# h3poteto/aws-global-accelerator-controller

Hardware: NVIDIA H100
Metric: objects reconciled/sec at 10^6 Service+Ingress; change-set bit-exact vs Go ref (higher is better)
Workload: dtype u8/u32 (bytes and indices)

## Files before the change

aws-global-accelerator-controller_b200/csrc/gar_common.h:

```cpp
#pragma once

#include <stdint.h>
#include <stddef.h>

#include "../../include/garecon.h"

#if defined(__CUDACC__)
#define GAR_HD __host__ __device__ __forceinline__
#define GAR_D __device__ __forceinline__
#else
#define GAR_HD inline
#define GAR_D inline
#endif

#if defined(__CUDA_ARCH__)
#define GAR_ANY(p) __any_sync(0xffffffffu, (p))
#else
bool gar_host_vote(bool p);
#define GAR_ANY(p) gar_host_vote((p))
#endif

typedef uint8_t u8;
typedef uint16_t u16;
typedef uint32_t u32;
// ... 102 lines not shown
#define XXP2 0xC2B2AE3D27D4EB4Full
#define XXP3 0x165667B19E3779F9ull
#define XXP4 0x85EBCA77C2B2AE63ull
#define XXP5 0x27D4EB2F165667C5ull

GAR_HD u64 rotl64(u64 x, int r) { return (x << r) | (x >> (64 - r)); }
GAR_HD u64 xx_round(u64 acc, u64 in) { return rotl64(acc + in * XXP2, 31) * XXP1; }
GAR_HD u64 xx_merge(u64 acc, u64 v) { return (acc ^ xx_round(0, v)) * XXP1 + XXP4; }
GAR_HD u64 xx_avalanche(u64 h) {
  h ^= h >> 33;
  h *= XXP2;
  h ^= h >> 29;
  h *= XXP3;
  h ^= h >> 32;
  return h;
}

GAR_HD u64 hash_init(u32 n) { return XXP5 ^ ((u64)n * XXP3); }
GAR_HD u64 hash_word(u64 h, u64 w) { return rotl64(h ^ (w * XXP2), 31) * XXP1 + XXP4; }
GAR_HD u64 load_word(Str s, u32 i) {
  u64 w = ld64u(s.p + i);
  if (s.n - i < 8) w &= lowmask(s.n - i);
  return w;
}
GAR_HD u64 gar_hash(Str s) {
  u64 h = hash_init(s.n);
  for (u32 i = 0; i < s.n; i += 8) h = hash_word(h, load_word(s, i));
  return xx_avalanche(h);
}

GAR_HD u64 u_hash(bool act, Str s) {
  u64 h = hash_init(s.n);
  const u32 n = act ? s.n : 0;
  for (u32 i = 0;; i += 8) {
    bool step = i < n;
    if (!GAR_ANY(step)) break;
    if (step) h = hash_word(h, load_word(s, i));
  }
  return xx_avalanche(h);
}
GAR_HD bool u_streq(bool act, Str a, Str b) {
  bool eq = act && a.n == b.n;
  const u32 n = eq ? a.n : 0;
  for (u32 i = 0;; i += 8) {
    bool step = eq && i < n;
    if (!GAR_ANY(step)) break;
    if (step) {
      u64 x = ld64u(a.p + i) ^ ld64u(b.p + i);
      if (n - i < 8) x &= lowmask(n - i);
      if (x) eq = false;
    }
  }
  return eq;
}
GAR_HD u32 u_find_byte(bool act, Str s, u32 from, u8 c) {
  u32 found = s.n;
  bool done = !act;
  for (u32 i = from;; i += 8) {
    bool step = !done && i < s.n;
    if (!GAR_ANY(step)) break;
    if (!step) continue;
    u64 m = swar_eq_mask(ld64u(s.p + i), c);
    if (s.n - i < 8) m &= lowmask(s.n - i);
    if (m) {
      found = i + (ctz64(m) >> 3);
      done = true;
    }
  }
  return found;
}

GAR_HD u64 hmix(u64 a, u64 b) { return xx_avalanche(a * XXP1 + rotl64(b, 29) * XXP2 + XXP5); }


struct alignas(32) IdxEntry {
  u32 tag, row, a0, a1;
  u64 s0, s1;
};

struct HashIdx {
  const u32 *begin;
  const IdxEntry *ent;
  u32 mask;
};

struct Cursor {
  u32 pos, end, tag;
};

GAR_HD u32 hash_bucket(u64 h, u32 mask) { return (u32)h & mask; }
GAR_HD u32 hash_tag(u64 h) { return (u32)(h >> 32); }

GAR_HD IdxEntry load_entry(const IdxEntry *p) {
#if defined(__CUDA_ARCH__)
  const uint4 *q = reinterpret_cast<const uint4 *>(p);
  uint4 lo = __ldg(q), hi = __ldg(q + 1);
  IdxEntry e;
  e.tag = lo.x;
  e.row = lo.y;
  e.a0 = lo.z;
  e.a1 = lo.w;
  e.s0 = (u64)hi.x | ((u64)hi.y << 32);
  e.s1 = (u64)hi.z | ((u64)hi.w << 32);
  return e;
#else
  return *p;
#endif
}

GAR_HD Cursor idx_open(const HashIdx &ix, u64 h) {
  u32 b = hash_bucket(h, ix.mask);
  Cursor c;
  c.pos = ix.begin[b];
  c.end = ix.begin[b + 1];
  c.tag = hash_tag(h);
  return c;
}
GAR_HD bool idx_next(const HashIdx &ix, Cursor &c, IdxEntry *out) {
  while (c.pos < c.end) {
    IdxEntry e = load_entry(ix.ent + c.pos++);
    if (e.tag == c.tag) {
      *out = e;
      return true;
    }
  }
  return false;
}
```

aws-global-accelerator-controller_b200/csrc/gar_pipeline.h:

```cpp
#pragma once

#include <stdio.h>
#include <stdlib.h>

#include <initializer_list>

#include "gar_rows.h"

#if defined(__CUDA_ARCH__)
#define GAR_ATOMIC_ADD(p, v) atomicAdd((p), (v))
#else
#define GAR_ATOMIC_ADD(p, v) (*(p) += (v))
#endif


enum Slot {
  S_DERIVED, S_OFLAGS, S_OKEY_HASH, S_STAGE_GA, S_STAGE_R53, S_ANN_R53, S_ANN_NAME, S_ANN_TAGS, S_ANN_LISTEN, S_DPORT_BEGIN, S_DPORTS,
  S_TOK_CODE, S_TOK_NAME, S_TOK_REGION,
  S_ACC_FLAGS, S_ACC_OWNER_KEY, S_ACC_OWNER, S_ACC_THOST, S_ACC_MANAGED, S_ACC_OWNER_HASH, S_ACC_THOST_HASH, S_REC_NAME_HASH, S_VAL_KEY_HASH,
  S_REC_ZONE, S_VAL_REC, S_VAL_CLS, S_VAL_KEY, S_VAL_ORPHAN, S_VAL_LINK, S_ACC_DIGEST,
  S_R53_MODE, S_R53_ACC, S_R53_ACC_DNS, S_PAIR_BEGIN, S_PAIR_OBJ, S_PAIR_HN, S_PAIR_CODE, S_PAIR_ZONE, S_PAIR_REC,
  S_IX_LB, S_IX_OWNER = S_IX_LB + 3, S_IX_THOST = S_IX_OWNER + 3, S_IX_ZONE = S_IX_THOST + 3, S_IX_VAL = S_IX_ZONE + 3,
  S_IX_ALIAS = S_IX_VAL + 3, S_IX_OBJ = S_IX_ALIAS + 3, S_IX_OVN = S_IX_OBJ + 3,
  S_SORT_KEYS = S_IX_OVN + 3, S_SORT_VALS, S_SORT_KEYS_ALT, S_SORT_VALS_ALT, S_SORT_TAGS,
// ... 283 lines not shown
    e->a1 = W.rec_zone[rec];
    e->s0 = T.a.rec_name[rec];
    e->s1 = T.a.val_value[v];
    return W.val_orphan[v] != 0;
  }
};

constexpr u32 IDX_SMALL_BUCKET = 48;
template <class RowF>
struct FIdxRows {
  RowF rowf;
  u32 *keys, *vals;
  IdxEntry *tmp;
  u32 *counts;
  u32 mask, nb;
  GAR_HD void operator()(u32 i) const {
    u64 h = 0;
    IdxEntry e;
    bool valid = rowf.make(i, &h, &e);
    u32 k = valid ? hash_bucket(h, mask) : nb;
    keys[i] = k;
    if (vals) vals[i] = i;
    if (valid) {
      e.tag = hash_tag(h);
      e.row = i;
      tmp[i] = e;
      GAR_ATOMIC_ADD(&counts[k], 1u);
    }
  }
};
struct FIdxPlace {
  const u32 *keys;
  u32 *cursor;
  const IdxEntry *tmp;
  IdxEntry *ent;
  u32 nb;
  GAR_HD void operator()(u32 i) const {
    u32 k = keys[i];
    if (k == nb) return;
#if defined(__CUDA_ARCH__)
    u32 pos = atomicAdd(&cursor[k], 1u);
#else
    u32 pos = cursor[k]++;
#endif
    ent[pos] = tmp[i];
  }
};
struct FIdxOrder {
  const u32 *begin;
  IdxEntry *ent;
  u32 *overflow;
  GAR_HD void operator()(u32 b) const {
    u32 lo = begin[b], m = begin[b + 1] - lo;
    if (m < 2) return;
    if (m > IDX_SMALL_BUCKET) {
      GAR_ATOMIC_ADD(overflow, 1u);
      return;
    }
    for (u32 k = 1; k < m; k++) {
      IdxEntry x = ent[lo + k];
      u32 j = k;
      while (j > 0 && ent[lo + j - 1].row > x.row) {
        ent[lo + j] = ent[lo + j - 1];
        j--;
      }
      if (j != k) ent[lo + j] = x;
    }
  }
};
struct FIdxGather {
  const u32 *vals;
  const u32 *nvalid;
  const IdxEntry *tmp;
  IdxEntry *ent;
  GAR_HD void operator()(u32 p) const {
    if (p < *nvalid) ent[p] = tmp[vals[p]];
  }
};
template <class RowF>
struct FIdxPlaceDirect {
  RowF rowf;
  u32 *cursor;
  IdxEntry *ent;
  u32 mask;
  GAR_HD void operator()(u32 i) const {
    u64 h = 0;
    IdxEntry e;
    if (!rowf.make(i, &h, &e)) return;
    const u32 k = hash_bucket(h, mask);
#if defined(__CUDA_ARCH__)
    const u32 pos = atomicAdd(&cursor[k], 1u);
#else
    const u32 pos = cursor[k]++;
#endif
    e.tag = hash_tag(h);
    e.row = i;
    ent[pos] = e;
  }
};
struct FIdxMultiList {
  const u32 *begin;
  u32 *multi;
  GAR_HD void operator()(u32 b) const {
    const bool m = begin[b + 1] - begin[b] >= 2;
#if defined(__CUDA_ARCH__)
    const unsigned active = __activemask();
    const unsigned votes = __ballot_sync(active, m);
    if (!m) return;
    const unsigned lane = threadIdx.x & 31u;
    const int leader = __ffs(votes) - 1;
    u32 base = 0;
    if ((int)lane == leader) base = atomicAdd(multi, (u32)__popc(votes));
    base = __shfl_sync(votes, base, leader);
    multi[1 + base + __popc(votes & ((1u << lane) - 1u))] = b;
#else
    if (m) multi[1 + multi[0]++] = b;
#endif
  }
};
struct FIdxOrderMulti {
  const u32 *begin;
  IdxEntry *ent;
  const u32 *multi;
  u32 *overflow;
  GAR_HD void operator()(u32 t) const {
    const u32 b = multi[1 + t];
    const u32 lo = begin[b], m = begin[b + 1] - lo;
    if (m > IDX_SMALL_BUCKET) {
      GAR_ATOMIC_ADD(overflow, 1u);
      return;
    }
    for (u32 k = 1; k < m; k++) {
      IdxEntry x = ent[lo + k];
      u32 j = k;
      while (j > 0 && ent[lo + j - 1].row > x.row) {
        ent[lo + j] = ent[lo + j - 1];
        j--;
      }
      if (j != k) ent[lo + j] = x;
    }
  }
};
enum FlagWord { FW_BAD_KEYS = 0, FW_IDX_OVERFLOW = 1, FW_NDPORTS = 2, FW_NPAIRS = 3, FW_SEC0 = 4 , FW_WORDS = 16 };
struct FGatherFinal {
  const u32 *src;
  u32 idx[5];
  const u32 *npairs;
  u32 *flags;
  GAR_HD void operator()(u32 k) const {
    if (k < 5) flags[FW_SEC0 + k] = src[idx[k]];
    else if (npairs) flags[FW_NPAIRS] = *npairs;
  }
};
struct FGather5 {
  const u32 *src;
  u32 idx[5];
  const u32 *extra;
  u32 *dst;
  GAR_HD void operator()(u32 k) const { dst[k] = k < 5 ? src[idx[k]] : *extra; }
};
#define GAR_RETRY_WITH_RADIX 1000
#define GAR_REFUSE_EMPTY_CACHE 1001
struct FGatherHeader {
  const u32 *ndports;
  u32 *flags;
  GAR_HD void operator()(u32) const { flags[FW_NDPORTS] = *ndports; }
};
struct FValueJoins {
  DevTables T;
  Work W;
  GAR_HD void operator()(u32 v) const {
    link_value_alias(T, W, v);
    mark_orphan_value(T, W, v);
  }
};
struct FMarkOrphanValue {
  DevTables T;
  Work W;
  GAR_HD void operator()(u32 v) const { mark_orphan_value(T, W, v); }
};

struct CountLayout {
  u32 n, nacc, nrec, nval;
  GAR_HD u32 ga_obj(u32 i) const { return i; }
  GAR_HD u32 ga_orph(u32 a) const { return n + a; }
  GAR_HD u32 r53_obj(u32 i) const { return n + nacc + i; }
  GAR_HD u32 base0() const { return 2 * n + nacc; }
  GAR_HD u32 base1() const { return 2 * n + nacc + nrec; }
  GAR_HD u32 total() const { return 2 * n + nacc + nrec + nval; }
};
constexpr u32 OPS_STAGE_CAP = 4;
struct FGaObj {
  DevTables T;
  Work W;
  u32 *counts;
  gar_op *stage;
  u32 *status;
  const u32 *rows;
  GAR_HD void operator()(u32 t, bool valid) const {
    u32 i = (rows && valid) ? rows[t] : t;
    OpSink s{stage + (size_t)t * OPS_STAGE_CAP, 0, OPS_STAGE_CAP};
    u32 st = ga_reconcile(T, W, i, valid, s);
    if (valid) {
      status[t] = st;
      counts[t] = s.n;
    }
  }
};
struct FR53Obj {
  DevTables T;
  Work W;
  u32 *counts;
  gar_op *stage;
  u32 *status;
  const u32 *rows;
  GAR_HD void operator()(u32 t, bool valid) const {
    u32 i = (rows && valid) ? rows[t] : t;
    OpSink s{stage + (size_t)t * OPS_STAGE_CAP, 0, OPS_STAGE_CAP};
    u32 prev = (valid && W.r53_mode[i] == R53_MODE_DONE) ? status[t] : 0;
    u32 st = r53_combine(T, W, i, t, valid, prev, s);
    if (valid) {
      status[t] = st;
      counts[t] = s.n;
// ... 151 lines not shown
    u32 zv = T.a.rec_val_begin[T.a.zone_rec_begin[z]];
    u32 off = counts[L.base0()] + (counts[L.base1() + zv] - counts[L.base1()]) + (counts[L.base0() + r] - counts[L.base0()]);
    OpSink s{ops + off, 0, 0xFFFFFFFFu};
    r53_orphan_alias(T, W, r, s);
  }
};
struct FR53OrphanValue {
  DevTables T;
  Work W;
  CountLayout L;
  u32 *counts;
  gar_op *ops;
  u32 cap;
  GAR_HD void operator()(u32 v) const {
    if (!ops) {
      counts[L.base1() + v] = W.val_orphan[v];
      return;
    }
    if (!W.val_orphan[v] || counts[L.total()] > cap) return;
    u32 r = W.val_rec[v];
    u32 z = W.rec_zone[r];
    u32 rend = T.a.zone_rec_begin[z + 1];
    u32 off = counts[L.base0()] + (counts[L.base0() + rend] - counts[L.base0()]) + (counts[L.base1() + v] - counts[L.base1()]);
    gar_op o;
    o.head = GAR_OP_HEAD(GAR_OP_R53_DELETE_RECORD, GAR_CTRL_R53, 0);
    o.obj = GAR_NONE;
    o.sub = 1;
    o.a0 = z;
    o.a1 = r;
    o.a2 = v;
    ops[off] = o;
  }
};


struct DiffCounts {
  u64 n_ops;
  u64 section_begin[GAR_N_SECTIONS + 1];
  u64 n_dports;
  u32 bad_keys;
};

GAR_HD u32 next_pow2(u32 x) {
  u32 p = 1;
  while (p < x) p <<= 1;
  return p;
}
inline int ilog2(u32 p) {
  int b = 0;
  while ((1u << b) < p) b++;
  return b;
}

template <class B>
struct Pipeline {
  B &be;
  DevTables T;
  Work W{};
  bool force_radix = false;
  explicit Pipeline(B &b, const DevTables &t) : be(b), T(t) {}

  template <class RowF>
  HashIdx build_index(int slot, u32 nrows, u32 load, RowF rowf, u32 *overflow, bool force_radix) {
    u32 nb = next_pow2(nrows / load < 16 ? 16 : nrows / load);
    u32 *keys = (u32 *)be.ensure(S_SORT_KEYS, sizeof(u32) * (size_t)(nrows + 1));
    u32 *vals = (u32 *)be.ensure(S_SORT_VALS, sizeof(u32) * (size_t)(nrows + 1));
    IdxEntry *tmp = (IdxEntry *)be.ensure(S_SORT_TAGS, sizeof(IdxEntry) * (size_t)(nrows + 1));
    u32 *begin = (u32 *)be.ensure(slot + 0, sizeof(u32) * (size_t)(nb + 2));
    IdxEntry *ent = (IdxEntry *)be.ensure(slot + 1, sizeof(IdxEntry) * (size_t)(nrows + 1));
    be.fill32(begin, 0, nb + 2);
    if (nrows) be.for_each("idx_rows", nrows, FIdxRows<RowF>{rowf, keys, force_radix ? vals : nullptr, tmp, begin, nb - 1, nb});
    be.exclusive_scan(begin, nb + 2);
    if (nrows && !force_radix) {
      u32 *cursor = (u32 *)be.ensure(S_SORT_KEYS_ALT, sizeof(u32) * (size_t)(nb + 1));
      be.copy32(cursor, begin, nb);
      be.for_each("idx_place", nrows, FIdxPlace{keys, cursor, tmp, ent, nb});
      be.for_each("idx_order", nb, FIdxOrder{begin, ent, overflow});
    } else if (nrows) {
      u32 *keys2 = (u32 *)be.ensure(S_SORT_KEYS_ALT, sizeof(u32) * (size_t)(nrows + 1));
      u32 *vals2 = (u32 *)be.ensure(S_SORT_VALS_ALT, sizeof(u32) * (size_t)(nrows + 1));
      be.sort_pairs(keys, vals, keys2, vals2, nrows, ilog2(nb) + 1);
      be.for_each("idx_gather", nrows, FIdxGather{vals, begin + nb, tmp, ent});
    }
    return HashIdx{begin, ent, nb - 1};
  }

  bool prepared = false;
  u64 n_dports = 0;
  u32 *errflag = nullptr;

  u32 acc_guest_from = 0xFFFFFFFFu;
  u32 sharded = 0;
  bool orphan_sweep = true;
  bool allow_empty_cache = false;

  void alloc_obj_work() {
    const u32 n = T.o.n_objects, nlbi = T.o.n_lbi;
    W.derived = (u32 *)be.ensure(S_DERIVED, 4 * (size_t)(n + 1));
    W.okey_hash = (u64 *)be.ensure(S_OKEY_HASH, 8 * (size_t)(n + 1));
    W.ann_r53 = (gar_str *)be.ensure(S_ANN_R53, 8 * (size_t)(n + 1));
    W.ann_name = (gar_str *)be.ensure(S_ANN_NAME, 8 * (size_t)(n + 1));
    W.ann_tags = (gar_str *)be.ensure(S_ANN_TAGS, 8 * (size_t)(n + 1));
    W.ann_listen = (gar_str *)be.ensure(S_ANN_LISTEN, 8 * (size_t)(n + 1));
    W.dport_begin = (u32 *)be.out_dport_begin(n);
    W.tok_code = (u8 *)be.out_tok_code(nlbi);
    W.tok_name = (gar_str *)be.out_tok_name(nlbi);
    W.tok_region = (gar_str *)be.out_tok_region(nlbi);
    W.r53_mode = (u8 *)be.ensure(S_R53_MODE, (size_t)n + 1);
    W.r53_acc = (u32 *)be.ensure(S_R53_ACC, 4 * (size_t)(n + 1));
    W.r53_acc_dns = (gar_str *)be.ensure(S_R53_ACC_DNS, 8 * (size_t)(n + 1));
  }
  void alloc_work() {
    const u32 nacc = T.a.n_accels, nrec = T.a.n_records, nval = T.a.n_values;
    alloc_obj_work();
    W.acc_flags = (u32 *)be.ensure(S_ACC_FLAGS, 4 * (size_t)(nacc + 1));
    W.acc_owner_key = (gar_str *)be.ensure(S_ACC_OWNER_KEY, 8 * (size_t)(nacc + 1));
    W.acc_owner = (gar_str *)be.ensure(S_ACC_OWNER, 8 * (size_t)(nacc + 1));
    W.acc_thost = (gar_str *)be.ensure(S_ACC_THOST, 8 * (size_t)(nacc + 1));
    W.acc_managed = (gar_str *)be.ensure(S_ACC_MANAGED, 8 * (size_t)(nacc + 1));
    W.acc_owner_hash = (u64 *)be.ensure(S_ACC_OWNER_HASH, 8 * (size_t)(nacc + 1));
    W.acc_thost_hash = (u64 *)be.ensure(S_ACC_THOST_HASH, 8 * (size_t)(nacc + 1));
    W.rec_name_hash = (u64 *)be.ensure(S_REC_NAME_HASH, 8 * (size_t)(nrec + 1));
    W.val_key_hash = (u64 *)be.ensure(S_VAL_KEY_HASH, 8 * (size_t)(nval + 1));
    W.rec_zone = (u32 *)be.ensure(S_REC_ZONE, 4 * (size_t)(nrec + 1));
    W.val_rec = (u32 *)be.ensure(S_VAL_REC, 4 * (size_t)(nval + 1));
    W.val_cls = (u8 *)be.ensure(S_VAL_CLS, nval + 1);
    W.val_key = (gar_str *)be.ensure(S_VAL_KEY, 8 * (size_t)(nval + 1));
    W.val_orphan = (u8 *)be.ensure(S_VAL_ORPHAN, nval + 1);
    W.val_link = (ValLink *)be.ensure(S_VAL_LINK, sizeof(ValLink) * (size_t)(nval + 1));
    W.acc_digest = (AccDigest *)be.ensure(S_ACC_DIGEST, sizeof(AccDigest) * (size_t)(nacc + 1));
    W.lb_hash = (u64 *)be.ensure(S_LB_HASH, 8 * (size_t)(T.a.n_lbs + 1));
    W.rec_flags = (u8 *)be.ensure(S_REC_FLAGS, (size_t)nrec + 1);
    for (int k = 0; k < IX_N; k++) W.hist[k] = IxHist{nullptr, 0};
    W.pair_cap = 0;
    W.dport_cap = 0;
    errflag = (u32 *)be.ensure(S_ERRFLAG, 256);
    be.fill32(errflag, 0, FW_WORDS);
    W.acc_guest_from = acc_guest_from;
    W.sharded = sharded;
    W.acc_claimed = nullptr;
  }
  void stage1() {
    const u32 n = T.o.n_objects, nlbi = T.o.n_lbi, nacc = T.a.n_accels, nrec = T.a.n_records, nval = T.a.n_values;
    u32 *derived_public = (u32 *)be.out_derived(n);
    if (n) be.for_each("classify_objects", n, FClassify{T, W, derived_public, nullptr, errflag});
    if (nlbi) be.for_each_staged("tokenise_hostnames", nlbi, FTokenise{T, W});
    if (nacc) be.for_each("digest_accelerators", nacc, FDigestAccel{T, W});
    if (T.a.n_lbs) be.for_each("hash_load_balancers", T.a.n_lbs, FLbHash{T, W});
    {
      unsigned long long *zm = (unsigned long long *)(errflag + 16 + 8);
      be.fill32((u32 *)zm, 0, 8);
      if (T.a.n_zones) be.for_each("zone_len_mask", T.a.n_zones, FZoneLenMask{T, W, zm});
      W.zone_len_mask = (const u64 *)zm;
    }
    if (nrec) {
      u32 *big = (u32 *)be.ensure(S_SORT_KEYS, 4 * (size_t)(nval / REC_INLINE_VALUES + 2));
      u32 *huge = (u32 *)be.ensure(S_SORT_VALS, 4 * (size_t)(nval / REC_HUGE_VALUES + 2));
      be.fill32(big, 0, 1);
      be.fill32(huge, 0, 1);
      be.for_each_staged("prepare_records", nrec, FPrepareRecord{T, W, big, huge});
      if (nval > REC_INLINE_VALUES) be.for_each("prepare_records", BIG_BLOCKS * 256, FClassifyBigRecords{T, W, big, huge});
    }
  }
  struct IxPlan {
    u32 off[IX_N] = {}, nb[IX_N] = {}, rows[IX_N] = {};
    bool want[IX_N] = {};
    u32 total_nb = 0;
    u64 total_rows = 0;
  };
  IxPlan planA;
  u32 *ixa_begin = nullptr, *ixa_fill = nullptr, *ixa_multi = nullptr;
  IdxEntry *ixa_ent = nullptr;
  u32 ovn_nb = 0;
  void arm_group_a(u32 want_mask) {
    const u32 rows[IX_N] = {T.a.n_lbs, T.a.n_accels, T.a.n_accels, T.a.n_zones, T.a.n_values, T.a.n_records, T.o.n_objects, 0};
    const u32 load[IX_N] = {1, 1, 1, 1, 1, 2, 1, 8};
    planA = IxPlan{};
    for (int k = 0; k < IX_OVN; k++) {
      planA.want[k] = (want_mask >> k) & 1u;
      if (!planA.want[k]) continue;
      planA.rows[k] = rows[k];
      planA.nb[k] = next_pow2(rows[k] / load[k] < 16 ? 16 : rows[k] / load[k]);
      planA.off[k] = planA.total_nb;
      planA.total_nb += planA.nb[k];
      planA.total_rows += rows[k];
    }
    ixa_begin = (u32 *)be.ensure(S_IXA_BEGIN, 4 * (size_t)(planA.total_nb + 2));
    be.fill32(ixa_begin, 0, (size_t)planA.total_nb + 2);
    for (int k = 0; k < IX_OVN; k++)
      if (planA.want[k]) W.hist[k] = IxHist{ixa_begin + planA.off[k], planA.nb[k] - 1};
  }
  HashIdx group_a_index(int k) const { return HashIdx{ixa_begin + planA.off[k], ixa_ent, planA.nb[k] - 1}; }
  template <class RowF>
  FIdxPlaceDirect<RowF> placer(int k, RowF rowf) const {
    return FIdxPlaceDirect<RowF>{rowf, ixa_fill + planA.off[k], ixa_ent, planA.nb[k] - 1};
  }
  void finish_group_a() {
    u32 *overflow = errflag + FW_IDX_OVERFLOW;
    be.exclusive_scan(ixa_begin, planA.total_nb + 1);
    ixa_fill = (u32 *)be.ensure(S_IXA_FILL, 4 * (size_t)(planA.total_nb + 1));
    ixa_ent = (IdxEntry *)be.ensure(S_IXA_ENT, sizeof(IdxEntry) * (size_t)(planA.total_rows + 1));
    const u32 multi_cap = (u32)(planA.total_rows / 2 + 1);
    ixa_multi = (u32 *)be.ensure(S_IXA_MULTI, 4 * (size_t)(multi_cap + 2));
    be.copy32(ixa_fill, ixa_begin, (size_t)planA.total_nb + 1);
    be.fill32(ixa_multi, 0, 1);
    const IxPlan &P = planA;
    auto n = [&](int k) { return P.want[k] ? P.rows[k] : 0u; };
    be.for_each_multi("idx_place", {n(IX_LB), n(IX_OWNER), n(IX_THOST), n(IX_ZONE), n(IX_VAL), n(IX_ALIAS), n(IX_OBJ), P.total_nb},
                      placer(IX_LB, FRowLb{T, W}), placer(IX_OWNER, FRowOwner{T, W}), placer(IX_THOST, FRowThost{T, W}), placer(IX_ZONE, FRowZone{T}),
                      placer(IX_VAL, FRowVal{T, W}), placer(IX_ALIAS, FRowAlias{T, W}), placer(IX_OBJ, FRowObj{T, W}), FIdxMultiList{ixa_begin, ixa_multi});
    be.for_each_dyn("idx_order", ixa_multi, multi_cap, FIdxOrderMulti{ixa_begin, ixa_ent, ixa_multi, overflow});
    if (P.want[IX_LB]) W.ix_lb = group_a_index(IX_LB);
    if (P.want[IX_OWNER]) W.ix_owner = group_a_index(IX_OWNER);
    if (P.want[IX_THOST]) W.ix_thost = group_a_index(IX_THOST);
    if (P.want[IX_ZONE]) W.ix_zone = group_a_index(IX_ZONE);
    if (P.want[IX_VAL]) W.ix_val = group_a_index(IX_VAL);
    if (P.want[IX_ALIAS]) W.ix_alias = group_a_index(IX_ALIAS);
    if (P.want[IX_OBJ]) W.ix_obj = group_a_index(IX_OBJ);
  }
  void arm_ovn() {
    ovn_nb = next_pow2(T.a.n_values / 8 < 16 ? 16 : T.a.n_values / 8);
    u32 *cnt = (u32 *)be.ensure(S_IX_OVN + 0, 4 * (size_t)(ovn_nb + 2));
    be.fill32(cnt, 0, (size_t)ovn_nb + 2);
    W.hist[IX_OVN] = IxHist{cnt, ovn_nb - 1};
  }
  void finish_ovn() {
    const u32 nval = T.a.n_values;
    u32 *begin = W.hist[IX_OVN].cnt;
    be.exclusive_scan(begin, ovn_nb + 1);
    u32 *cursor = (u32 *)be.ensure(S_OVN_FILL, 4 * (size_t)(ovn_nb + 1));
    IdxEntry *ent = (IdxEntry *)be.ensure(S_IX_OVN + 1, sizeof(IdxEntry) * (size_t)(nval + 1));
    u32 *multi = (u32 *)be.ensure(S_OVN_MULTI, 4 * (size_t)(nval / 2 + 3));
    be.copy32(cursor, begin, (size_t)ovn_nb + 1);
    be.fill32(multi, 0, 1);
    be.for_each_multi("idx_place", {nval, ovn_nb}, FIdxPlaceDirect<FRowOvn>{FRowOvn{T, W}, cursor, ent, ovn_nb - 1}, FIdxMultiList{begin, multi});
    be.for_each_dyn("idx_order", multi, nval / 2 + 1, FIdxOrderMulti{begin, ent, multi, errflag + FW_IDX_OVERFLOW});
    W.ix_ovn = HashIdx{begin, ent, ovn_nb - 1};
  }

  void prepare_route() {
    alloc_work();
    arm_group_a(1u << IX_ALIAS);
    stage1();
    finish_group_a();
  }
  void prepare_directory() {
    alloc_work();
    arm_group_a((1u << IX_LB) | (1u << IX_THOST));
    if (T.o.n_lbi) be.for_each("tokenise_hostnames", T.o.n_lbi, FTokenise{T, W});
    if (T.a.n_accels) be.for_each("digest_accelerators", T.a.n_accels, FDigestAccel{T, W});
    if (T.a.n_lbs) be.for_each("hash_load_balancers", T.a.n_lbs, FLbHash{T, W});
    finish_group_a();
  }

  u32 dport_cap = 0, pair_cap = 0;
  u64 ops_cap = 0;
  bool tiny_caps = false;
  int prepare() {
    const u32 n = T.o.n_objects, nacc = T.a.n_accels, nzone = T.a.n_zones, nrec = T.a.n_records, nval = T.a.n_values;
    alloc_work();
    if (!force_radix) {
      arm_group_a((1u << IX_OVN) - 1);
      arm_ovn();
    }
    stage1();
    listen_ports();

    u32 *overflow = errflag + FW_IDX_OVERFLOW;
    if (!force_radix) {
      finish_group_a();
      if (nval) be.for_each("value_joins", nval, FValueJoins{T, W});
      finish_ovn();
    } else {
      W.ix_lb = build_index(S_IX_LB, T.a.n_lbs, 1, FRowLb{T, W}, overflow, true);
      W.ix_owner = build_index(S_IX_OWNER, nacc, 1, FRowOwner{T, W}, overflow, true);
      W.ix_thost = build_index(S_IX_THOST, nacc, 1, FRowThost{T, W}, overflow, true);
      W.ix_zone = build_index(S_IX_ZONE, nzone, 1, FRowZone{T}, overflow, true);
      W.ix_val = build_index(S_IX_VAL, nval, 1, FRowVal{T, W}, overflow, true);
      W.ix_alias = build_index(S_IX_ALIAS, nrec, 2, FRowAlias{T, W}, overflow, true);
      W.ix_obj = build_index(S_IX_OBJ, n, 1, FRowObj{T, W}, overflow, true);
      if (nval) be.for_each("value_joins", nval, FValueJoins{T, W});
      W.ix_ovn = build_index(S_IX_OVN, nval, 8, FRowOvn{T, W}, overflow, true);
    }
    obj_stale = ovn_stale = false;
    return GAR_OK;
  }
  void listen_ports() {
    const u32 n = T.o.n_objects;
    be.fill32(W.dport_begin, 0, (size_t)n + 1);
    if (n) be.for_each("listen_ports_count", n, FJsonCount{T, W});
    be.exclusive_scan(W.dport_begin, n + 1);
    be.for_each("gather_header", 1, FGatherHeader{W.dport_begin + n, errflag});
    if (dport_cap < n / 2 + 1024 && !(tiny_caps && dport_cap)) dport_cap = tiny_caps ? 1 : n / 2 + 1024;
    W.dport_cap = dport_cap;
    W.dports = (i32 *)be.out_dports(dport_cap);
    if (n) be.for_each("listen_ports_write", n, FJsonWrite{T, W});
  }

  bool obj_stale = false, ovn_stale = false;
  void prepare_objects() {
    const u32 n = T.o.n_objects, nlbi = T.o.n_lbi;
    alloc_obj_work();
    be.fill32(errflag, 0, FW_WORDS);
    W.hist[IX_OBJ] = IxHist{nullptr, 0};
    u32 *derived_public = (u32 *)be.out_derived(n);
    if (n) be.for_each("classify_objects", n, FClassify{T, W, derived_public, nullptr, errflag});
    if (nlbi) be.for_each_staged("tokenise_hostnames", nlbi, FTokenise{T, W});
    listen_ports();
    W.ix_obj = build_index(S_IX_OBJ, n, 1, FRowObj{T, W}, errflag + FW_IDX_OVERFLOW, force_radix);
    obj_stale = false;
    ovn_stale = true;
  }
  void prepare_orphan_values() {
    const u32 nval = T.a.n_values;
    if (!force_radix) {
      arm_ovn();
      if (nval) be.for_each("orphan_values", nval, FMarkOrphanValue{T, W});
      finish_ovn();
    } else {
      W.hist[IX_OVN] = IxHist{nullptr, 0};
// ... 192 lines not shown
```

aws-global-accelerator-controller_b200/csrc/gar_rows.h:

```cpp
#pragma once

#include "gar_common.h"
#include "gar_json.h"


struct DevTables {
  gar_objects o;
  gar_actual a;
  const u8 *cluster;
  u32 cluster_len;
};

enum {
  OBJ_HAS_NAME_ANN = 1u << 8,
  OBJ_HAS_TAGS_ANN = 1u << 9,
  OBJ_KEY_BAD = 1u << 10,
};

enum {
  ACC_MINE = 1u << 0,
  ACC_OWNER_KEYED = 1u << 1,
  ACC_OWNER_INGRESS = 1u << 2,
  ACC_OWNER_3PART = 1u << 3,
  ACC_HAS_MANAGED = 1u << 4, ACC_HAS_OWNER = 1u << 5, ACC_HAS_THOST = 1u << 6,
// ... 950 lines not shown
    const AccDigest d = W.acc_digest[acc];
    const bool created = (d.flags & (ACCD_LIS_NONE | ACCD_EG_NONE)) != 0;
    bool replaced = created;
    for (u32 jp = 0; jp < j && !replaced; jp++) {
      if (W.tok_code[jb + jp] > GAR_TOK_NLB) continue;
      u32 st;
      u32 lbp = find_lb(T, W, mkstr(T.o.slab, W.tok_region[jb + jp]), mkstr(T.o.slab, W.tok_name[jb + jp]), &st);
      if (lbp != GAR_NONE && !eg_contains(T, d, mkstr(A.slab, A.lb_arn[lbp]))) replaced = true;
    }
    const bool contains = replaced ? !arn_differs : eg_contains(T, d, lb_arn);
    if (!contains) s.put(GAR_OP_HEAD(GAR_OP_GA_UPDATE_EG, GAR_CTRL_GA, kind), i, j, acc, created ? GAR_PENDING : d.eg, lb);
  }
}


constexpr u32 OWNED_CACHE = 8;
struct OwnedHit {
  u32 v, rec, zone;
  gar_str name;
};
struct Owned {
  OwnedHit hit[OWNED_CACHE];
  u32 n;
  u64 okh;
  u32 kind;
  Str key;
};
GAR_HD bool owned_match(const DevTables &T, const IdxEntry &e, u32 kind, Str key) {
  return (e.a1 >> 31) == kind && streq(mkstr(T.a.slab, e.s0), key);
}
GAR_HD void owned_collect(const DevTables &T, const Work &W, u64 okh, u32 kind, Str key, Owned &o) {
  o.n = 0;
  o.okh = okh;
  o.kind = kind;
  o.key = key;
  Cursor c = idx_open(W.ix_val, okh);
  IdxEntry e;
  while (idx_next(W.ix_val, c, &e)) {
    if (!owned_match(T, e, kind, key)) continue;
    if (o.n < OWNED_CACHE) o.hit[o.n] = OwnedHit{e.row, e.a0, e.a1 & 0x3FFFFFFFu, e.s1};
    o.n++;
  }
}
GAR_HD void u_owned_collect(const DevTables &T, const Work &W, bool active, u64 okh, u32 kind, Str key, Owned &o) {
  if (active) {
    o.n = 0;
    o.okh = okh;
    o.kind = kind;
    o.key = key;
  }
  Cursor c = active ? idx_open(W.ix_val, okh) : Cursor{0, 0, 0};
  for (; GAR_ANY(c.pos < c.end);) {
    IdxEntry e;
    bool hit = false;
    if (c.pos < c.end) {
      e = load_entry(W.ix_val.ent + c.pos++);
      hit = e.tag == c.tag && (e.a1 >> 31) == kind;
    }
    if (u_streq(hit, hit ? mkstr(T.a.slab, e.s0) : Str{T.a.slab, 0}, key)) {
      if (o.n < OWNED_CACHE) o.hit[o.n] = OwnedHit{e.row, e.a0, e.a1 & 0x3FFFFFFFu, e.s1};
      o.n++;
    }
  }
}
GAR_HD OwnedHit owned_get(const DevTables &T, const Work &W, const Owned &o, u32 k) {
  if (k < OWNED_CACHE) return o.hit[k];
  Cursor c = idx_open(W.ix_val, o.okh);
  IdxEntry e;
  u32 seen = 0;
  OwnedHit h{GAR_NONE, GAR_NONE, GAR_NONE, 0};
  while (idx_next(W.ix_val, c, &e)) {
    if (!owned_match(T, e, o.kind, o.key)) continue;
    if (seen++ == k) {
      h = OwnedHit{e.row, e.a0, e.a1 & 0x3FFFFFFFu, e.s1};
      break;
    }
  }
  return h;
}

GAR_HD u32 first_alias_a(const DevTables &T, const Work &W, u32 zone, Str name, u64 name_hash, gar_str *alias_dns) {
  Cursor c = idx_open(W.ix_alias, key_hash_zoned_h(zone, name_hash));
  IdxEntry e;
  while (idx_next(W.ix_alias, c, &e)) {
    if (e.a0 != zone || e.a1 != GAR_RR_A) continue;
    if (streq(mkstr(T.a.slab, e.s0), name)) {
      *alias_dns = e.s1;
      return e.row;
    }
  }
  return GAR_NONE;
}
GAR_HD u32 next_alias_any(const DevTables &T, const Work &W, u32 zone, Str name, u32 after ) {
  Cursor c = idx_open(W.ix_alias, key_hash_zoned(zone, name));
  IdxEntry e;
  while (idx_next(W.ix_alias, c, &e)) {
    if (after != GAR_NONE && e.row <= after) continue;
    if (e.a0 != zone) continue;
    if (streq(mkstr(T.a.slab, e.s0), name)) return e.row;
  }
  return GAR_NONE;
}

GAR_HD void r53_cleanup(const DevTables &T, const Work &W, u32 obj, u32 kind, const Owned &ow, OpSink &s) {
  const gar_actual &A = T.a;
  u32 head = GAR_OP_HEAD(GAR_OP_R53_DELETE_RECORD, GAR_CTRL_R53, obj == GAR_NONE ? 0 : kind);
  u32 k = 0;
  while (k < ow.n) {
    u32 zone = owned_get(T, W, ow, k).zone;
    u32 kend = k;
    while (kend < ow.n && owned_get(T, W, ow, kend).zone == zone) kend++;
    u32 last = GAR_NONE;
    for (;;) {
      u32 best = GAR_NONE, best_v = GAR_NONE;
      for (u32 x = k; x < kend; x++) {
        OwnedHit h = owned_get(T, W, ow, x);
        u32 r = next_alias_any(T, W, zone, mkstr(A.slab, h.name), last);
        if (r != GAR_NONE && (best == GAR_NONE || r < best)) {
          best = r;
          best_v = h.v;
        }
      }
      if (best == GAR_NONE) break;
      s.put(head, obj, 0, zone, best, best_v);
      last = best;
    }
    for (u32 x = k; x < kend; x++) {
      OwnedHit h = owned_get(T, W, ow, x);
      s.put(head, obj, 1, zone, h.rec, h.v);
    }
    k = kend;
  }
}

GAR_HD bool piece_seen_before(Str all, Str hn) {
  u32 pos = 0;
  Str piece;
  while (next_piece(all, &pos, &piece)) {
    if (piece.p >= hn.p) return false;
    if (streq(piece, hn)) return true;
  }
  return false;
}

GAR_HD u32 r53_reconcile(const DevTables &T, const Work &W, u32 i, bool valid, OpSink &s) {
  const gar_objects &o = T.o;
  const gar_actual &A = T.a;
  u32 result = GAR_STATUS(GAR_ST_IGNORED, 0, 0);
  u32 kind = 0, jb = 0, nj = 0;
  Str okey{T.o.slab, 0}, hostnames{T.o.slab, 0};
  u64 okh = 0;
  bool ensure = false;
  Owned ow;
  ow.n = 0;
  if (valid) {
    u32 dv = W.derived[i];
    if (dv & GAR_DV_R53_ELIGIBLE) {
      kind = o.obj_kind[i];
      okey = object_key(T, i);
      okh = W.okey_hash[i];
      if (!(dv & GAR_DV_R53_ANNOTATED)) {
        owned_collect(T, W, okh, kind, okey, ow);
        r53_cleanup(T, W, i, kind, ow, s);
        result = GAR_STATUS(GAR_ST_OK, 0, GAR_EV_DELETED);
      } else {
        ensure = true;
        hostnames = mkstr(o.slab, W.ann_r53[i]);
        jb = o.obj_lbi_begin[i];
        nj = o.obj_lbi_begin[i + 1] - jb;
// ... 206 lines not shown
  u32 i = 0, kind = 0;
  Str hn{T.o.slab, 0}, okey{T.o.slab, 0};
  u64 okh = 0;
  valid = valid && W.pair_code[p] != PAIR_REPEAT;
  if (valid) {
    i = W.pair_obj[p];
    hn = mkstr(T.o.slab, W.pair_hn[p]);
    kind = T.o.obj_kind[i];
    okey = object_key(T, i);
    okh = W.okey_hash[i];
  }
  u32 zone = u_find_hosted_zone(T, W, valid, hn);
  bool live = valid && zone != GAR_NONE;
  u32 rec = GAR_NONE;
  gar_str rec_alias = 0;
  Cursor c = u_open(W.ix_val, live, okh);
  for (; GAR_ANY(c.pos < c.end);) {
    IdxEntry e;
    bool hit = false;
    if (c.pos < c.end) {
      e = load_entry(W.ix_val.ent + c.pos++);
      hit = e.tag == c.tag && (e.a1 >> 31) == kind && (e.a1 & 0x3FFFFFFFu) == zone;
    }
    bool mine = u_streq(hit, hit ? mkstr(A.slab, e.s0) : Str{A.slab, 0}, okey);
    Str nm = mine ? mkstr(A.slab, e.s1) : Str{A.slab, 0};
    bool plain = mine && !(e.a1 & VALNAME_HAS_BACKSLASH);
    bool shape = plain && nm.n == hn.n + 1 && nm.p[nm.n - 1] == '.';
    bool match = u_streq(shape, substr(nm, 0, shape ? hn.n : 0), hn);
    if (mine && !plain) match = record_name_matches(nm, hn);
    if (match) {
      ValLink l = W.val_link[e.row];
      if (l.alias_row != GAR_NONE && (rec == GAR_NONE || l.alias_row < rec)) {
        rec = l.alias_row;
        rec_alias = l.alias_dns;
      }
    }
  }
  bool have = live && rec != GAR_NONE;
  Str acc_dns = have ? mkstr(A.slab, W.r53_acc_dns[i]) : Str{A.slab, 0};
  Str al = have ? mkstr(A.slab, rec_alias) : Str{A.slab, 0};
  bool shape = have && al.n == acc_dns.n + 1 && al.p[al.n - 1] == '.';
  bool same = u_streq(shape, substr(al, 0, shape ? acc_dns.n : 0), acc_dns);
  if (valid) {
    u32 code = !live ? PAIR_NO_ZONE : rec == GAR_NONE ? PAIR_CREATE : same ? PAIR_IN_SYNC : PAIR_UPSERT;
    W.pair_code[p] = (u8)code;
    W.pair_zone[p] = zone;
    W.pair_rec[p] = rec;
  }
}

GAR_HD u32 r53_combine(const DevTables &T, const Work &W, u32 i, u32 t, bool valid, u32 prev_status, OpSink &s) {
  u32 mode = valid ? W.r53_mode[i] : R53_MODE_DONE;
  u32 st = prev_status;
  bool slow = mode == R53_MODE_OBJECT;
  if (GAR_ANY(slow)) {
    u32 r = r53_reconcile(T, W, i, slow, s);
    if (slow) st = r;
  }
  if (mode == R53_MODE_PAIRS) {
    u32 kind = T.o.obj_kind[i], acc = W.r53_acc[i];
    bool created = false, stop = false;
    u32 k = 0;
    for (u32 p = W.pair_begin[t]; p < W.pair_begin[t + 1] && p < W.pair_cap && !stop; p++, k++) {
      u32 code = W.pair_code[p];
      if (code == PAIR_NO_ZONE) {
        st = GAR_STATUS(GAR_ST_ERR_RETRY, GAR_D_NO_HOSTED_ZONE, 0);
        stop = true;
      } else if (code == PAIR_CREATE) {
        s.put(GAR_OP_HEAD(GAR_OP_R53_CREATE, GAR_CTRL_R53, kind), i, GAR_R53_SUB(0, k), W.pair_zone[p], acc, GAR_NONE);
        created = true;
      } else if (code == PAIR_UPSERT) {
        s.put(GAR_OP_HEAD(GAR_OP_R53_UPSERT_A, GAR_CTRL_R53, kind), i, GAR_R53_SUB(0, k), W.pair_zone[p], acc, W.pair_rec[p]);
      }
    }
    if (!stop) st = GAR_STATUS(GAR_ST_OK, 0, created ? GAR_EV_CREATED : 0);
  }
  return st;
}


GAR_HD bool object_in_cache(const DevTables &T, const Work &W, u32 kind, Str key, u64 key_hash) {
  Cursor c = idx_open(W.ix_obj, key_hash);
  IdxEntry e;
  while (idx_next(W.ix_obj, c, &e))
    if (e.a0 == kind && streq(mkstr(T.o.slab, e.s0), key)) return true;
  return false;
}

GAR_HD u32 ga_orphan(const DevTables &T, const Work &W, u32 acc, OpSink &s) {
  if (acc >= W.acc_guest_from) return 0;
  if (W.acc_claimed && W.acc_claimed[acc]) return 0;
  u32 fl = W.acc_flags[acc];
  if (!(fl & ACC_MINE) || !(fl & ACC_OWNER_3PART)) return 0;
  u32 kind = (fl & ACC_OWNER_INGRESS) ? 1u : 0u;
  if (object_in_cache(T, W, kind, mkstr(T.a.slab, W.acc_owner_key[acc]), W.acc_owner_hash[acc])) return 0;
  put_delete_chain(T, s, GAR_NONE, 0, acc);
  return 1;
}

GAR_HD void mark_orphan_value(const DevTables &T, const Work &W, u32 v) {
  u32 cls = W.val_cls[v];
  u8 orphan = 0;
  if (cls & VAL_OWNER_3PART) {
    u32 kind = (cls & VAL_OWNER_INGRESS) ? 1u : 0u;
    orphan = object_in_cache(T, W, kind, mkstr(T.a.slab, W.val_key[v]), W.val_key_hash[v]) ? 0 : 1;
  }
  if (orphan) {
    u32 rec = W.val_rec[v];
    ix_count(W.hist[IX_OVN], key_hash_zoned_h(W.rec_zone[rec], W.rec_name_hash[rec]));
  }
  W.val_orphan[v] = orphan;
}

GAR_HD void r53_orphan_alias(const DevTables &T, const Work &W, u32 r, OpSink &s) {
  const gar_actual &A = T.a;
  if (!A.rec_has_alias[r]) return;
  u32 zone = W.rec_zone[r];
  Str name = mkstr(A.slab, A.rec_name[r]);
  u64 h = key_hash_zoned_h(zone, W.rec_name_hash[r]);
  Cursor c = idx_open(W.ix_ovn, h);
  IdxEntry e;
  while (idx_next(W.ix_ovn, c, &e)) {
    if (e.a1 != zone || !streq(mkstr(A.slab, e.s0), name)) continue;
    Str val = mkstr(A.slab, e.s1);
    bool dup = false;
    Cursor c2 = idx_open(W.ix_ovn, h);
    IdxEntry e2;
    while (idx_next(W.ix_ovn, c2, &e2) && e2.row < e.row) {
      if (e2.a1 == zone && streq(mkstr(A.slab, e2.s0), name) && streq(mkstr(A.slab, e2.s1), val)) {
        dup = true;
        break;
      }
    }
    if (dup) continue;
    s.put(GAR_OP_HEAD(GAR_OP_R53_DELETE_RECORD, GAR_CTRL_R53, 0), GAR_NONE, 0, zone, r, e.row);
  }
}


struct DevBindings {
  gar_bindings b;
  HashIdx ix_eg;
};

GAR_HD bool egb_eg_exists(const DevBindings &B, Str arn) {
  Cursor c = idx_open(B.ix_eg, gar_hash(arn));
  IdxEntry e;
  while (idx_next(B.ix_eg, c, &e))
    if (streq(mkstr(B.b.slab, e.s0), arn)) return true;
  return false;
}

GAR_HD u32 egb_lb_of(const DevTables &T, const Work &W, u32 lbi_row, u32 *detail) {
  u32 code = W.tok_code[lbi_row];
  *detail = 0;
  if (code == GAR_TOK_NOT_AWS || code == GAR_TOK_PANIC) {
    *detail = GAR_D_NOT_ELB;
    return GAR_NONE;
  }
  if (code >= GAR_TOK_ERR_NOT_ELB) {
    *detail = GAR_D_NOT_ELB + (code - GAR_TOK_ERR_NOT_ELB);
    return GAR_NONE;
  }
  u32 st;
  u32 lb = find_lb(T, W, mkstr(T.o.slab, W.tok_region[lbi_row]), mkstr(T.o.slab, W.tok_name[lbi_row]), &st);
  if (lb == GAR_NONE) *detail = GAR_D_LB_NOT_FOUND;
  return lb;
}
// ... 99 lines not shown
```

Before: 165.7 million.

## Inline first 32 key bytes into widened object-index entries

The object-cache hash index now uses 64-byte entries, and the first 32 bytes of each key are copied next to the entry when it is placed. Lookups in object_in_cache (and first_alias_a, if its index is wide) compare against these inline bytes, so a probe no longer needs a dependent gather into the object slab. Wide entries are loaded with an L2 64B prefetch hint. In exchange the object index takes twice the memory and placement writes more, the bucket-ordering pass moves double-size units, and the per-index allocation order changes so the object index comes first.

```diff
diff --git a/aws-global-accelerator-controller_b200/csrc/gar_common.h b/aws-global-accelerator-controller_b200/csrc/gar_common.h
--- a/aws-global-accelerator-controller_b200/csrc/gar_common.h
+++ b/aws-global-accelerator-controller_b200/csrc/gar_common.h
@@ -208,6 +208,7 @@
   const u32 *begin;
   const IdxEntry *ent;
   u32 mask;
+  u32 wide;
 };
 
 struct Cursor {
@@ -217,10 +218,20 @@
 GAR_HD u32 hash_bucket(u64 h, u32 mask) { return (u32)h & mask; }
 GAR_HD u32 hash_tag(u64 h) { return (u32)(h >> 32); }
 
-GAR_HD IdxEntry load_entry(const IdxEntry *p) {
+GAR_HD const IdxEntry *idx_entry(const HashIdx &ix, u32 pos) { return ix.ent + ((size_t)pos << ix.wide); }
+GAR_HD u32 idx_inline_cap(const HashIdx &ix) { return ix.wide ? 32u : 0u; }
+
+GAR_HD IdxEntry load_entry(const IdxEntry *p, u32 wide = 0) {
 #if defined(__CUDA_ARCH__)
   const uint4 *q = reinterpret_cast<const uint4 *>(p);
-  uint4 lo = __ldg(q), hi = __ldg(q + 1);
+  uint4 lo, hi;
+  if (wide) {
+    asm("ld.global.nc.L2::64B.v4.u32 {%0,%1,%2,%3}, [%4];" : "=r"(lo.x), "=r"(lo.y), "=r"(lo.z), "=r"(lo.w) : "l"(q));
+    asm("ld.global.nc.L2::64B.v4.u32 {%0,%1,%2,%3}, [%4];" : "=r"(hi.x), "=r"(hi.y), "=r"(hi.z), "=r"(hi.w) : "l"(q + 1));
+  } else {
+    lo = __ldg(q);
+    hi = __ldg(q + 1);
+  }
   IdxEntry e;
   e.tag = lo.x;
   e.row = lo.y;
@@ -242,13 +253,36 @@
   c.tag = hash_tag(h);
   return c;
 }
-GAR_HD bool idx_next(const HashIdx &ix, Cursor &c, IdxEntry *out) {
+GAR_HD bool idx_next(const HashIdx &ix, Cursor &c, IdxEntry *out, const IdxEntry **at = nullptr) {
   while (c.pos < c.end) {
-    IdxEntry e = load_entry(ix.ent + c.pos++);
+    const IdxEntry *p = idx_entry(ix, c.pos++);
+    IdxEntry e = load_entry(p, ix.wide);
     if (e.tag == c.tag) {
       *out = e;
+      if (at) *at = p;
       return true;
     }
   }
   return false;
 }
+
+GAR_HD u64 inline_word(const IdxEntry *p, u32 cap, Str s, u32 i) {
+  if (i + 8 <= cap) {
+    const u64 *q = reinterpret_cast<const u64 *>(p + 1) + (i >> 3);
+#if defined(__CUDA_ARCH__)
+    return (u64)__ldg(reinterpret_cast<const unsigned long long *>(q));
+#else
+    return *q;
+#endif
+  }
+  return ld64u(s.p + i);
+}
+GAR_HD bool inline_eq(const IdxEntry *p, u32 cap, Str stored, Str key) {
+  if (stored.n != key.n) return false;
+  for (u32 i = 0; i < key.n; i += 8) {
+    u64 x = inline_word(p, cap, stored, i) ^ ld64u(key.p + i);
+    if (key.n - i < 8) x &= lowmask(key.n - i);
+    if (x) return false;
+  }
+  return true;
+}
diff --git a/aws-global-accelerator-controller_b200/csrc/gar_pipeline.h b/aws-global-accelerator-controller_b200/csrc/gar_pipeline.h
--- a/aws-global-accelerator-controller_b200/csrc/gar_pipeline.h
+++ b/aws-global-accelerator-controller_b200/csrc/gar_pipeline.h
@@ -389,11 +389,18 @@
   RowF rowf;
   u32 *cursor;
   IdxEntry *ent;
-  u32 mask;
+  u32 mask, wide;
+  const u8 *slab;
   GAR_HD void operator()(u32 i) const {
     u64 h = 0;
     IdxEntry e;
     if (!rowf.make(i, &h, &e)) return;
+    const Str key = mkstr(slab, e.s0);
+    u64 w[4];
+#if defined(__CUDA_ARCH__)
+#pragma unroll
+#endif
+    for (u32 j = 0; j < 4; j++) w[j] = wide && 8 * j < key.n ? load_word(key, 8 * j) : 0ull;
     const u32 k = hash_bucket(h, mask);
 #if defined(__CUDA_ARCH__)
     const u32 pos = atomicAdd(&cursor[k], 1u);
@@ -402,7 +409,16 @@
 #endif
     e.tag = hash_tag(h);
     e.row = i;
-    ent[pos] = e;
+    IdxEntry *p = ent + ((size_t)pos << wide);
+    *p = e;
+    if (!wide) return;
+    u64 *inl = reinterpret_cast<u64 *>(p + 1);
+#if defined(__CUDA_ARCH__)
+    reinterpret_cast<uint4 *>(inl)[0] = make_uint4((u32)w[0], (u32)(w[0] >> 32), (u32)w[1], (u32)(w[1] >> 32));
+    reinterpret_cast<uint4 *>(inl)[1] = make_uint4((u32)w[2], (u32)(w[2] >> 32), (u32)w[3], (u32)(w[3] >> 32));
+#else
+    for (u32 j = 0; j < 4; j++) inl[j] = w[j];
+#endif
   }
 };
 struct FIdxMultiList {
@@ -425,11 +441,30 @@
 #endif
   }
 };
+template <u32 U>
+struct EntryUnits {
+  IdxEntry u[U];
+};
+template <u32 U>
+GAR_HD void order_bucket(IdxEntry *base, u32 m) {
+  EntryUnits<U> *ent = reinterpret_cast<EntryUnits<U> *>(base);
+  for (u32 k = 1; k < m; k++) {
+    EntryUnits<U> x = ent[k];
+    u32 j = k;
+    while (j > 0 && ent[j - 1].u[0].row > x.u[0].row) {
+      ent[j] = ent[j - 1];
+      j--;
+    }
+    if (j != k) ent[j] = x;
+  }
+}
 struct FIdxOrderMulti {
   const u32 *begin;
   IdxEntry *ent;
   const u32 *multi;
   u32 *overflow;
+  u32 wide_nb;
+  IdxEntry *wide_ent;
   GAR_HD void operator()(u32 t) const {
     const u32 b = multi[1 + t];
     const u32 lo = begin[b], m = begin[b + 1] - lo;
@@ -437,15 +472,8 @@
       GAR_ATOMIC_ADD(overflow, 1u);
       return;
     }
-    for (u32 k = 1; k < m; k++) {
-      IdxEntry x = ent[lo + k];
-      u32 j = k;
-      while (j > 0 && ent[lo + j - 1].row > x.row) {
-        ent[lo + j] = ent[lo + j - 1];
-        j--;
-      }
-      if (j != k) ent[lo + j] = x;
-    }
+    if (b < wide_nb) order_bucket<2>(wide_ent + 2 * (size_t)lo, m);
+    else order_bucket<1>(ent + lo, m);
   }
 };
 enum FlagWord { FW_BAD_KEYS = 0, FW_IDX_OVERFLOW = 1, FW_NDPORTS = 2, FW_NPAIRS = 3, FW_SEC0 = 4 , FW_WORDS = 16 };
@@ -763,7 +791,7 @@
       be.sort_pairs(keys, vals, keys2, vals2, nrows, ilog2(nb) + 1);
       be.for_each("idx_gather", nrows, FIdxGather{vals, begin + nb, tmp, ent});
     }
-    return HashIdx{begin, ent, nb - 1};
+    return HashIdx{begin, ent, nb - 1, 0};
   }
 
   bool prepared = false;
@@ -851,13 +879,14 @@
   };
   IxPlan planA;
   u32 *ixa_begin = nullptr, *ixa_fill = nullptr, *ixa_multi = nullptr;
-  IdxEntry *ixa_ent = nullptr;
+  IdxEntry *ixa_ent = nullptr, *ixa_obj_ent = nullptr;
   u32 ovn_nb = 0;
   void arm_group_a(u32 want_mask) {
     const u32 rows[IX_N] = {T.a.n_lbs, T.a.n_accels, T.a.n_accels, T.a.n_zones, T.a.n_values, T.a.n_records, T.o.n_objects, 0};
     const u32 load[IX_N] = {1, 1, 1, 1, 1, 2, 1, 8};
+    const int order[IX_OVN] = {IX_OBJ, IX_LB, IX_OWNER, IX_THOST, IX_ZONE, IX_VAL, IX_ALIAS};
     planA = IxPlan{};
-    for (int k = 0; k < IX_OVN; k++) {
+    for (int k : order) {
       planA.want[k] = (want_mask >> k) & 1u;
       if (!planA.want[k]) continue;
       planA.rows[k] = rows[k];
@@ -871,16 +900,21 @@
     for (int k = 0; k < IX_OVN; k++)
       if (planA.want[k]) W.hist[k] = IxHist{ixa_begin + planA.off[k], planA.nb[k] - 1};
   }
-  HashIdx group_a_index(int k) const { return HashIdx{ixa_begin + planA.off[k], ixa_ent, planA.nb[k] - 1}; }
+  HashIdx group_a_index(int k) const {
+    return k == IX_OBJ ? HashIdx{ixa_begin + planA.off[k], ixa_obj_ent, planA.nb[k] - 1, 1} : HashIdx{ixa_begin + planA.off[k], ixa_ent, planA.nb[k] - 1, 0};
+  }
   template <class RowF>
   FIdxPlaceDirect<RowF> placer(int k, RowF rowf) const {
-    return FIdxPlaceDirect<RowF>{rowf, ixa_fill + planA.off[k], ixa_ent, planA.nb[k] - 1};
+    const HashIdx ix = group_a_index(k);
+    return FIdxPlaceDirect<RowF>{rowf, ixa_fill + planA.off[k], const_cast<IdxEntry *>(ix.ent), ix.mask, ix.wide, k == IX_OBJ ? T.o.slab : T.a.slab};
   }
   void finish_group_a() {
     u32 *overflow = errflag + FW_IDX_OVERFLOW;
     be.exclusive_scan(ixa_begin, planA.total_nb + 1);
     ixa_fill = (u32 *)be.ensure(S_IXA_FILL, 4 * (size_t)(planA.total_nb + 1));
-    ixa_ent = (IdxEntry *)be.ensure(S_IXA_ENT, sizeof(IdxEntry) * (size_t)(planA.total_rows + 1));
+    const size_t narrow_units = ((size_t)planA.total_rows + 1 + 3) & ~(size_t)3;
+    ixa_ent = (IdxEntry *)be.ensure(S_IXA_ENT, sizeof(IdxEntry) * (narrow_units + 2 * ((size_t)planA.rows[IX_OBJ] + 1)));
+    ixa_obj_ent = ixa_ent + narrow_units;
     const u32 multi_cap = (u32)(planA.total_rows / 2 + 1);
     ixa_multi = (u32 *)be.ensure(S_IXA_MULTI, 4 * (size_t)(multi_cap + 2));
     be.copy32(ixa_fill, ixa_begin, (size_t)planA.total_nb + 1);
@@ -890,7 +924,7 @@
     be.for_each_multi("idx_place", {n(IX_LB), n(IX_OWNER), n(IX_THOST), n(IX_ZONE), n(IX_VAL), n(IX_ALIAS), n(IX_OBJ), P.total_nb},
                       placer(IX_LB, FRowLb{T, W}), placer(IX_OWNER, FRowOwner{T, W}), placer(IX_THOST, FRowThost{T, W}), placer(IX_ZONE, FRowZone{T}),
                       placer(IX_VAL, FRowVal{T, W}), placer(IX_ALIAS, FRowAlias{T, W}), placer(IX_OBJ, FRowObj{T, W}), FIdxMultiList{ixa_begin, ixa_multi});
-    be.for_each_dyn("idx_order", ixa_multi, multi_cap, FIdxOrderMulti{ixa_begin, ixa_ent, ixa_multi, overflow});
+    be.for_each_dyn("idx_order", ixa_multi, multi_cap, FIdxOrderMulti{ixa_begin, ixa_ent, ixa_multi, overflow, P.nb[IX_OBJ], ixa_obj_ent});
     if (P.want[IX_LB]) W.ix_lb = group_a_index(IX_LB);
     if (P.want[IX_OWNER]) W.ix_owner = group_a_index(IX_OWNER);
     if (P.want[IX_THOST]) W.ix_thost = group_a_index(IX_THOST);
@@ -914,9 +948,10 @@
     u32 *multi = (u32 *)be.ensure(S_OVN_MULTI, 4 * (size_t)(nval / 2 + 3));
     be.copy32(cursor, begin, (size_t)ovn_nb + 1);
     be.fill32(multi, 0, 1);
-    be.for_each_multi("idx_place", {nval, ovn_nb}, FIdxPlaceDirect<FRowOvn>{FRowOvn{T, W}, cursor, ent, ovn_nb - 1}, FIdxMultiList{begin, multi});
-    be.for_each_dyn("idx_order", multi, nval / 2 + 1, FIdxOrderMulti{begin, ent, multi, errflag + FW_IDX_OVERFLOW});
-    W.ix_ovn = HashIdx{begin, ent, ovn_nb - 1};
+    be.for_each_multi("idx_place", {nval, ovn_nb}, FIdxPlaceDirect<FRowOvn>{FRowOvn{T, W}, cursor, ent, ovn_nb - 1, 0, T.a.slab},
+                      FIdxMultiList{begin, multi});
+    be.for_each_dyn("idx_order", multi, nval / 2 + 1, FIdxOrderMulti{begin, ent, multi, errflag + FW_IDX_OVERFLOW, 0, nullptr});
+    W.ix_ovn = HashIdx{begin, ent, ovn_nb - 1, 0};
   }
 
   void prepare_route() {
diff --git a/aws-global-accelerator-controller_b200/csrc/gar_rows.h b/aws-global-accelerator-controller_b200/csrc/gar_rows.h
--- a/aws-global-accelerator-controller_b200/csrc/gar_rows.h
+++ b/aws-global-accelerator-controller_b200/csrc/gar_rows.h
@@ -1056,9 +1056,10 @@
 GAR_HD u32 first_alias_a(const DevTables &T, const Work &W, u32 zone, Str name, u64 name_hash, gar_str *alias_dns) {
   Cursor c = idx_open(W.ix_alias, key_hash_zoned_h(zone, name_hash));
   IdxEntry e;
-  while (idx_next(W.ix_alias, c, &e)) {
+  const IdxEntry *at;
+  while (idx_next(W.ix_alias, c, &e, &at)) {
     if (e.a0 != zone || e.a1 != GAR_RR_A) continue;
-    if (streq(mkstr(T.a.slab, e.s0), name)) {
+    if (inline_eq(at, idx_inline_cap(W.ix_alias), mkstr(T.a.slab, e.s0), name)) {
       *alias_dns = e.s1;
       return e.row;
     }
@@ -1431,8 +1432,9 @@
 GAR_HD bool object_in_cache(const DevTables &T, const Work &W, u32 kind, Str key, u64 key_hash) {
   Cursor c = idx_open(W.ix_obj, key_hash);
   IdxEntry e;
-  while (idx_next(W.ix_obj, c, &e))
-    if (e.a0 == kind && streq(mkstr(T.o.slab, e.s0), key)) return true;
+  const IdxEntry *at;
+  while (idx_next(W.ix_obj, c, &e, &at))
+    if (e.a0 == kind && inline_eq(at, idx_inline_cap(W.ix_obj), mkstr(T.o.slab, e.s0), key)) return true;
   return false;
 }
 
```

New measurement: 169.2 million, median of 6. 2.1% higher.
